# Cobalt-27/CompactFusion

Measured on AMD Instinct MI355X. Metric: residual_compressed_activation_exchange_throughput, higher is better.
Workload: dtype f16

## Files before the change

compactfusion_amd/csrc/cfx_absmean.hip:

```cpp
#include <hip/hip_runtime.h>
#include <hip/hip_ext.h>
#include <stdint.h>
#include <stdio.h>
#include <stdlib.h>
#include <string.h>
#include <algorithm>
#include "cfx.h"
#include "cfx_internal.h"
#include "cfx_device.h"
#include "cfx_host.h"

#define CFX_I_FLAG_LR_FACTORS_ONLY 0x100
#define CFX_I_FLAG_LR_ABS 0x200
extern "C" CFX_HIDDEN size_t cfx_i_lr_workspace_bytes_any(int N, int C, int rank, int batch);
extern "C" CFX_HIDDEN void cfx_i_lr_factor_offsets(int N, int C, int rank, size_t* offU16, size_t* offV16, size_t* per);

template <bool EMIT_BITS, int US, bool WT = false, int NW = WAVES, bool PUB = false, bool KEEP = false, bool TAG = false>
__device__ __forceinline__ void absmean_stats_body(const cfx_comp_item& it, int N, int C, int R, int CB, int bx, int by,
                                                   u64* rowpart, u64 (*sm)[TILE_C], Probe probe = Probe(),
                                                   h16x8* xk = nullptr, h16x8* bk = nullptr, TagArena ta = TagArena()) {
#define SSTAMP(k) probe.at(k)
    const TileCoord t = tile_coord_at(bx, by, N, C, R);
    const int cb = bx;
    u64* colpart = rowpart + (size_t)N * CB;
// ... 250 lines not shown
        for (int e = 0; e < 8; ++e) acc[j][e] = 0.f;
    for (int k0 = 0; k0 < K; k0 += 8) {
        h16 v[8][8];
#pragma unroll
        for (int e = 0; e < 8; ++e)
#pragma unroll
            for (int k = 0; k < 8; ++k) v[e][k] = (k0 + k < K) ? VT[(size_t)(t.c + e) * K + k0 + k] : (h16)0;
#pragma unroll
        for (int j = 0; j < RPT; ++j) {
            const int r = t.r0 + t.w + j * WAVES;
            if (r >= t.r1) continue;
            h16 u[8];
#pragma unroll
            for (int k = 0; k < 8; ++k) u[k] = (k0 + k < K) ? U[(size_t)r * K + k0 + k] : (h16)0;
#pragma unroll
            for (int e = 0; e < 8; ++e)
#pragma unroll
                for (int k = 0; k < 8; ++k) acc[j][e] += (float)(h16)(u[k] * v[e][k]);
        }
    }
#pragma unroll
    for (int j = 0; j < RPT; ++j) {
        const int r = t.r0 + t.w + j * WAVES;
        if (r >= t.r1) continue;
        h16x8 bv = (h16x8)(h16)0, xv = (h16x8)(h16)0;
        if (base) bv = ld8(base + (size_t)r * C + t.c);
        unsigned byte;
        if (QUANT) {
            xv = ld8(x + (size_t)r * C + t.c);
            const h16x8 d = xv - bv;
            byte = 0;
#pragma unroll
            for (int i = 0; i < 8; ++i) byte |= (d[i] >= (h16)0 ? 1u : 0u) << i;
            pk[(size_t)r * C8 + (t.c >> 3)] = (unsigned char)byte;
        } else byte = pk[(size_t)r * C8 + (t.c >> 3)];
        if (!upd) continue;
        h16x8 o;
#pragma unroll
        for (int e = 0; e < 8; ++e) {
            const h16 sc = (h16)acc[j][e];
            const h16 recv = ((byte >> e) & 1u) ? sc : -sc;
            o[e] = base ? (h16)(bv[e] + recv) : recv;
        }
        if (QUANT && !ef) o = xv;
        st8(out + (size_t)r * C + t.c, o);
    }
}

#ifndef WATCH_SLEEP
#define WATCH_SLEEP 4
#endif
#ifndef INT2_FLAG_SLEEP
#define INT2_FLAG_SLEEP 2
#endif
__device__ __forceinline__ void scales_watch(const TagArena& ta, int N, int C, int c0, int r0, long long timeout) {
    const int tid = threadIdx.x;
    if (tid < 2) {
        const u64* w = tid ? ta.tU + min(r0, N - 1) : ta.tV + min(c0 + ((r0 >> 1) & (TILE_C - 1)), C - 1);
        SpinClock clk;
        while (!tag_is(ld_wt(w), ta.tagbits)) {
            __builtin_amdgcn_s_sleep(WATCH_SLEEP);
            if (clk.expired(timeout)) break;
        }
    }
    lds_barrier();
}
template <int ROWS, bool WATCH = true>
__device__ __forceinline__ bool scales_from_tagged(const TagArena& ta, int N, int C, int c0, int r0, u16* s16, long long timeout, unsigned* err) {
    static_assert(ROWS <= TILE_C, "one token word per thread (512 threads = the column block's channels)");
    const int tid = threadIdx.x;
    const u64* pv = ta.tV + min(c0 + tid, C - 1);
    const u64* pu = ta.tU + min(r0 + tid, N - 1);
    SpinClock clk;
    if (WATCH) scales_watch(ta, N, C, c0, r0, timeout);
    for (;;) {
        const u64 v = ld_wt(pv);
        const u64 u = tid < ROWS ? ld_wt(pu) : ta.tagbits;
        const bool ok = tag_is(v, ta.tagbits) && tag_is(u, ta.tagbits);
        s16[tid] = (u16)v;
        if (tid < ROWS) s16[TILE_C + tid] = (u16)u;
        if (!__syncthreads_or(ok ? 0 : 1)) return true;
        __builtin_amdgcn_s_sleep(2);
        if (__syncthreads_or(!ok && clk.expired(timeout) ? 1 : 0)) {
            if (tid == 0) gate_fail(err);
            return false;
        }
    }
}

#ifndef ONEBIT_D_TAGGED
#define ONEBIT_D_TAGGED 0
#endif
template <int NW, int KR, int KL, bool ST>
__device__ __forceinline__ void binary_dequant_gated_body(const cfx_decomp_item& it, int N, int C, int R, int tile_x, int tile_y,
                                                         unsigned* gate, unsigned expect, unsigned* err, long long timeout, u32x4* lds,
                                                         Probe probe = Probe(), bool remote = false, bool tagged = false, TagArena ta = TagArena(),
                                                         u16* s16 = nullptr) {
    constexpr int K = KR + KL;
#define GSTAMP(k) do { if (ST && probe.on()) { asm volatile("s_waitcnt vmcnt(0)" ::: "memory"); probe.at(k); } } while (0)
    const TileCoord t = tile_coord_at(tile_x, tile_y, N, C, R);
    if (ST) { probe.at(0); probe.set(7, 4); }
    const unsigned char* pk = (const unsigned char*)it.packet;
    const int C8 = C >> 3;
    const u16* U = (const u16*)(pk + (size_t)N * C8);
    const u16* V = U + N;
    const h16* base = (const h16*)it.base;
    h16* out = (h16*)it.recon;
    const int cc = min(t.c, C - 8);
    h16x8 bv[KR];
    if (base) {
#pragma unroll
        for (int j = 0; j < KR; ++j) bv[j] = ld8nt(base + (size_t)min(t.r0 + t.w + NW * j, t.r1 - 1) * C + cc);
        if constexpr (KL > 0) {
            h16x8 tl[KL > 0 ? KL : 1];
#pragma unroll
            for (int j = 0; j < KL; ++j) tl[j] = ld8nt(base + (size_t)min(t.r0 + t.w + NW * (KR + j), t.r1 - 1) * C + cc);
#pragma unroll
            for (int j = 0; j < KL; ++j) lds[j * (NW * 64) + threadIdx.x] = __builtin_bit_cast(u32x4, tl[j]);
        }
    } else {
#pragma unroll
        for (int j = 0; j < KR; ++j) bv[j] = (h16x8)(h16)0;
    }
    GSTAMP(1);
    h16x8 v8;
    u16 ul;
    unsigned by[K];
    if (tagged) {
        scales_watch(ta, N, C, tile_x * TILE_C, t.r0, timeout);
        if (ST) probe.at(2);
#pragma unroll
        for (int j = 0; j < K; ++j) by[j] = ld_wt(pk + (size_t)min(t.r0 + t.w + NW * j, t.r1 - 1) * C8 + (cc >> 3));
        if (!scales_from_tagged<NW * K, false>(ta, N, C, tile_x * TILE_C, t.r0, s16, timeout, err)) return;
        v8 = __builtin_bit_cast(h16x8, *(const u16x8*)(s16 + 8 * t.lane));
        ul = s16[TILE_C + min(t.w + NW * min(t.lane, K - 1), t.r1 - 1 - t.r0)];
    } else if (!gate_wait<true>(gate, expect, err, timeout)) return;
    else if (remote) {
        if (ST) probe.at(2);
        u16x8 vb;
#pragma unroll
        for (int i = 0; i < 8; ++i) vb[i] = ld_sys(V + cc + i);
        v8 = __builtin_bit_cast(h16x8, vb);
        ul = ld_sys(U + min(t.r0 + t.w + NW * min(t.lane, K - 1), t.r1 - 1));
#pragma unroll
        for (int j = 0; j < K; ++j) by[j] = ld_sys(pk + (size_t)min(t.r0 + t.w + NW * j, t.r1 - 1) * C8 + (cc >> 3));
    } else {
        if (ST) probe.at(2);
        v8 = ld8_wt(V + cc);
        ul = ld_wt(U + min(t.r0 + t.w + NW * min(t.lane, K - 1), t.r1 - 1));
#pragma unroll
        for (int j = 0; j < K; ++j) by[j] = ld_wt(pk + (size_t)min(t.r0 + t.w + NW * j, t.r1 - 1) * C8 + (cc >> 3));
    }
    GSTAMP(3);
#pragma unroll
    for (int j = 0; j < K; ++j) {
        const int rr = t.r0 + t.w + NW * j;
        const h16 uj = hfrom((u16)__builtin_amdgcn_readlane((int)ul, j));
        if (rr < t.r1 && t.act) {
            const h16x8 s = v8 * uj;
            u16x8 sb = __builtin_bit_cast(u16x8, s);
#pragma unroll
            for (int i = 0; i < 8; ++i) sb[i] ^= ((by[j] >> i) & 1u) ? (u16)0 : (u16)0x8000;
            const h16x8 recv = __builtin_bit_cast(h16x8, sb);
            h16x8 bj = (h16x8)(h16)0;
            if (j < KR) bj = bv[j < KR ? j : 0];
            else if (base) bj = __builtin_bit_cast(h16x8, lds[(j - KR) * (NW * 64) + threadIdx.x]);
            st8nt(out + (size_t)rr * C + t.c, base ? (bj + recv) : recv);
        }
    }
    GSTAMP(4);
#undef GSTAMP
}

__device__ __forceinline__ void row_sums2_wt(const u64* rowpart, const unsigned* row32, int N, int CB, int m0, int m1, bool two, u64& s0, u64& s1) {
    s0 = 0; s1 = 0;
    for (int k0 = 0; k0 < CB; k0 += FUSED_RCH) {
        unsigned a[FUSED_RCH], b[FUSED_RCH];
#pragma unroll
        for (int j = 0; j < FUSED_RCH; ++j) a[j] = ld_wt(&row32[(size_t)min(k0 + j, CB - 1) * N + m0]);
        if (two) {
#pragma unroll
            for (int j = 0; j < FUSED_RCH; ++j) b[j] = ld_wt(&row32[(size_t)min(k0 + j, CB - 1) * N + m1]);
        } else {
#pragma unroll
            for (int j = 0; j < FUSED_RCH; ++j) b[j] = 0;
        }
        bool sat = false;
#pragma unroll
        for (int j = 0; j < FUSED_RCH; ++j) {
            s0 += (k0 + j < CB) ? a[j] : 0; s1 += (k0 + j < CB) ? b[j] : 0;
            sat |= (a[j] == PART_SAT) | (b[j] == PART_SAT);
        }
        if (sat) {
            for (int j = 0; j < FUSED_RCH && k0 + j < CB; ++j) {
                if (a[j] == PART_SAT) s0 += ld_wt(&rowpart[(size_t)(k0 + j) * N + m0]) - (u64)PART_SAT;
                if (two && b[j] == PART_SAT) s1 += ld_wt(&rowpart[(size_t)(k0 + j) * N + m1]) - (u64)PART_SAT;
            }
        }
    }
}

template <bool GATED>
__device__ __forceinline__ void absmean_last_arriver_jobs(const cfx_comp_item& it, int N, int C, int CB, int P, int bx, u64* rowpart,
                                                          unsigned* tick, int per_byte, int eps_mode, u64 (*sm)[TILE_C], bool last_col,
                                                          bool last_all, Probe probe, unsigned* gate, unsigned gate_expect) {
    constexpr int NT = FUSED_NT;
#define STAMP(k) probe.at(k)
    lds_barrier();
    const int tid = threadIdx.x;
    const u64* colpart = rowpart + (size_t)N * CB;
    const unsigned* row32 = part32_of(rowpart, N, C, CB);
    const unsigned* col32 = row32 + (size_t)N * CB;
    h16* U = (h16*)((char*)it.packet + (size_t)N * (C / per_byte));
    h16* V = U + N;
    const int c = bx * TILE_C + tid;
    const int cc = min(c, C - 1);
    unsigned v[FUSED_CH];
    if (last_col) {
#pragma unroll
        for (int j = 0; j < FUSED_CH; ++j) v[j] = ld_wt(&col32[(size_t)min(j, P - 1) * C + cc]);
    }
    u64 keep0 = 0, keep1 = 0;
    if (last_all) row_sums2_wt(rowpart, row32, N, CB, min(tid, N - 1), min(tid + NT, N - 1), (tid & ~63) + NT < N, keep0, keep1);
    asm volatile("" ::: "memory");
    STAMP(4);
    u64* smem = &sm[1][0];
    float m0 = 0.f, m1 = 0.f;
    if (last_all) {
        const h16 h0 = mean16(keep0, C), h1 = mean16(keep1, C);
        m0 = (float)h0; m1 = (float)h1;
        u64 acc = 0;
        if (tid < N) acc += habs_units(hbits(h0));
        if (tid + NT < N) acc += habs_units(hbits(h1));
        for (int n0 = tid + 2 * NT; n0 - tid < N; n0 += 2 * NT) {
            const int n1 = n0 + NT;
            u64 s0, s1;
            row_sums2_wt(rowpart, row32, N, CB, min(n0, N - 1), min(n1, N - 1), (n1 & ~63) < N, s0, s1);
            if (n0 < N) acc += habs_units(hbits(mean16(s0, C)));
            if (n1 < N) acc += habs_units(hbits(mean16(s1, C)));
        }
        STAMP(13);
        u64 wtot;
        if (N <= 2 * NT) {
            const unsigned lo = wave_sum_u32_dpp((unsigned)(acc & 0xffffffu));
            const unsigned hi = wave_sum_u32_dpp((unsigned)(acc >> 24));
            wtot = ((u64)hi << 24) + lo;
        } else wtot = wave_sum_u64(acc);
        STAMP(14);
        if ((tid & 63) == 0) smem[tid >> 6] = wtot;
    }
    h16 vmean = (h16)0;
    if (last_col) {
        u64 a = 0;
        for (int p0 = 0; p0 < P; p0 += FUSED_CH) {
            if (p0) {
#pragma unroll
                for (int j = 0; j < FUSED_CH; ++j) v[j] = ld_wt(&col32[(size_t)min(p0 + j, P - 1) * C + cc]);
            }
            bool sat = false;
#pragma unroll
            for (int j = 0; j < FUSED_CH; ++j) { a += (p0 + j < P) ? v[j] : 0; sat |= v[j] == PART_SAT; }
            if (sat) {
                for (int j = 0; j < FUSED_CH && p0 + j < P; ++j)
                    if (v[j] == PART_SAT) a += ld_wt(&colpart[(size_t)(p0 + j) * C + cc]) - (u64)PART_SAT;
            }
        }
        vmean = mean16(a, N);
    }
    STAMP(5);
    if (last_all) {
        lds_barrier();
        STAMP(15);
        u64 tot = 0;
#pragma unroll
        for (int w = 0; w < NT / 64; ++w) tot += smem[w];
        const h16 mu = mean16(tot, N);
        const float den = eps_mode ? (float)(h16)((float)mu + 1e-6f) : (float)mu;
#define PUT16(ptr, val) do { const h16 _v = (val); if (GATED) st_wt((u16*)(ptr), hbits(_v)); else *(ptr) = _v; } while (0)
        if (tid < N) PUT16(&U[tid], (h16)(m0 / den));
        if (tid + NT < N) PUT16(&U[tid + NT], (h16)(m1 / den));
        for (int n0 = tid + 2 * NT; n0 - tid < N; n0 += 2 * NT) {
            const int n1 = n0 + NT;
            u64 s0, s1;
            row_sums2_wt(rowpart, row32, N, CB, min(n0, N - 1), min(n1, N - 1), (n1 & ~63) < N, s0, s1);
            if (n0 < N) PUT16(&U[n0], (h16)((float)mean16(s0, C) / den));
            if (n1 < N) PUT16(&U[n1], (h16)((float)mean16(s1, C) / den));
        }
        if (tid == 0) st_wt(tick + TICK_ALL, 0u);
    }
    if (last_col) {
        if (c < C) PUT16(&V[c], vmean);
        if (tid == 0) st_wt(tick + 1 + bx, 0u);
    }
#undef PUT16
    if (GATED) {
        asm volatile("s_waitcnt vmcnt(0)" ::: "memory");
        lds_barrier();
        if (tid == 0) gate_arrive_few(gate, (last_all ? 1u : 0u) + (last_col ? 1u : 0u));
    }
    STAMP(6);
#undef STAMP
}

__device__ __forceinline__ void absmean_tagged_jobs(const cfx_comp_item& it, int N, int C, int CB, int P, int bx, u64* rowpart, const TagArena& ta,
                                                    int per_byte, int eps_mode, u64 (*sm)[TILE_C], bool do_col, bool do_row, Probe probe,
                                                    unsigned* gate, unsigned* err, long long timeout) {
    constexpr int NT = FUSED_NT;
#define STAMP(k) probe.at(k)
    lds_barrier();
    const int tid = threadIdx.x;
    const u64* colpart = rowpart + (size_t)N * CB;
    h16* U = (h16*)((char*)it.packet + (size_t)N * (C / per_byte));
    h16* V = U + N;
    SpinClock clk;
    bool failed = false;
#define PUT16(ptr, val) st_wt((u16*)(ptr), hbits(val))
    if (do_col) {
        const int c = bx * TILE_C + tid, cc = min(c, C - 1);
        u64 a = 0;
        for (int p0 = 0; p0 < P && !failed; p0 += FUSED_CH) {
            u64 v[FUSED_CH];
            for (;;) {
#pragma unroll
                for (int j = 0; j < FUSED_CH; ++j) v[j] = ld_wt(&ta.tcol[(size_t)min(p0 + j, P - 1) * C + cc]);
                bool ok = true;
#pragma unroll
                for (int j = 0; j < FUSED_CH; ++j) ok = ok && tag_is(v[j], ta.tagbits);
                if (ok) break;
                __builtin_amdgcn_s_sleep(2);
                if (clk.expired(timeout)) { failed = true; break; }
            }
#pragma unroll
            for (int j = 0; j < FUSED_CH; ++j) {
                const u64 w = v[j] & TAG_SAT;
                if (p0 + j < P) a += (w == TAG_SAT && !failed) ? ld_wt(&colpart[(size_t)(p0 + j) * C + cc]) : w;
            }
        }
        STAMP(4);
        failed = __syncthreads_or(failed ? 1 : 0) != 0;
        if (!failed) {
            if (c < C) {
                const h16 vm = mean16(a, N);
                st_wt(&ta.tV[c], ta.tagbits | (u64)hbits(vm));
                PUT16(&V[c], vm);
            }
            asm volatile("s_waitcnt vmcnt(0)" ::: "memory");
            lds_barrier();
            if (tid == 0) gate_arrive_few(gate, 1u);
        }
        STAMP(5);
    }
    if (do_row && !failed) {
        u64* smem = &sm[1][0];
        auto row_sum = [&](int n) {
            const int nc = min(n, N - 1);
            u64 s_ = 0;
            for (int k0 = 0; k0 < CB && !failed; k0 += FUSED_RCH) {
                u64 q[FUSED_RCH];
                for (;;) {
#pragma unroll
                    for (int j = 0; j < FUSED_RCH; ++j) q[j] = ld_wt(&ta.trow[(size_t)min(k0 + j, CB - 1) * N + nc]);
                    bool ok = true;
#pragma unroll
                    for (int j = 0; j < FUSED_RCH; ++j) ok = ok && tag_is(q[j], ta.tagbits);
                    if (ok) break;
                    __builtin_amdgcn_s_sleep(2);
                    if (clk.expired(timeout)) { failed = true; break; }
                }
#pragma unroll
                for (int j = 0; j < FUSED_RCH; ++j) {
                    const u64 w = q[j] & TAG_SAT;
                    if (k0 + j < CB) s_ += (w == TAG_SAT && !failed) ? ld_wt(&rowpart[(size_t)(k0 + j) * N + nc]) : w;
                }
            }
            return s_;
        };
        h16 h0 = (h16)0, h1 = (h16)0;
        u64 acc = 0;
        for (int n0 = tid, i = 0; n0 - tid < N; n0 += NT, ++i) {
            const h16 h = mean16(row_sum(n0), C);
            if (i == 0) h0 = h;
            if (i == 1) h1 = h;
            if (n0 < N) acc += habs_units(hbits(h));
        }
        STAMP(13);
        const u64 wtot = wave_sum_u64(acc);
        if ((tid & 63) == 0) smem[tid >> 6] = wtot;
        failed = __syncthreads_or(failed ? 1 : 0) != 0;
        STAMP(15);
        if (!failed) {
            u64 tot = 0;
#pragma unroll
            for (int w = 0; w < NT / 64; ++w) tot += smem[w];
            const h16 mu = mean16(tot, N);
            const float den = eps_mode ? (float)(h16)((float)mu + 1e-6f) : (float)mu;
            for (int n0 = tid, i = 0; n0 < N; n0 += NT, ++i) {
                const h16 h = i == 0 ? h0 : (i == 1 ? h1 : mean16(row_sum(n0), C));
                const h16 un = (h16)((float)h / den);
                st_wt(&ta.tU[n0], ta.tagbits | (u64)hbits(un));
                PUT16(&U[n0], un);
            }
            asm volatile("s_waitcnt vmcnt(0)" ::: "memory");
            lds_barrier();
            if (tid == 0) gate_arrive_few(gate, 1u);
        }
        STAMP(6);
    }
#undef PUT16
#undef STAMP
    if (failed && tid == 0) gate_fail(err);
}

template <int US>
__device__ __forceinline__ void own_tile_finish(const cfx_comp_item& it, int N, int C, int R, int bx, int by, int flags, const h16x8* xk,
                                                const h16x8* bk, unsigned* gate1, unsigned expect1, unsigned* gate2, unsigned expect2,
                                                unsigned* err, long long timeout, unsigned char* smw, const TagArena& ta, u16* s16) {
    constexpr int NW = FUSED_NW;
    static_assert(US * 8 <= 64, "a wave publishes its US rows of codes with 8 lanes a row");
    const TileCoord t = tile_coord_at(bx, by, N, C, R);
    h16* nb = (h16*)it.new_base;
    const bool upd = (flags & CFX_FLAG_UPDATE_CACHE) && nb;
    const bool ef = !(flags & CFX_FLAG_NO_EF);
    unsigned char* pk = (unsigned char*)it.packet;
    (void)gate1; (void)expect1;
    if (!scales_from_tagged<NW * US>(ta, N, C, bx * TILE_C, t.r0, s16, timeout, err)) return;
    const h16x8 ch8 = __builtin_bit_cast(h16x8, *(const u16x8*)(s16 + 8 * t.lane));
    const u16 ul = s16[TILE_C + min(t.w + NW * min(t.lane, US - 1), t.r1 - 1 - t.r0)];
    const bool has_base = it.base != nullptr;
    u16 codes[US];
#pragma unroll
    for (int j = 0; j < US; ++j) {
        const int rr = t.r0 + t.w + NW * j;
        const h16 tk = hfrom((u16)__builtin_amdgcn_readlane((int)ul, j));
        codes[j] = 0;
        if (rr < t.r1 && t.act) {
            const h16x8 d = xk[j] - bk[j];
            const h16x8 thr = ch8 * tk;
            const h16x8 a = habs8(d);
            unsigned code = 0;
#pragma unroll
            for (int i = 0; i < 8; ++i) {
                const unsigned sg = d[i] >= (h16)0 ? 1u : 0u;
                const unsigned m = a[i] > thr[i] ? 1u : 0u;
                code |= ((sg << 1) | m) << (2 * i);
            }
            codes[j] = (u16)code;
            ((u16*)smw)[j * 64 + t.lane] = (u16)code;
        }
    }
    {
        const int j = t.lane >> 3, seg = t.lane & 7;
        const int rr = t.r0 + t.w + NW * j;
        if (t.lane < 8 * US && rr < t.r1 && bx * TILE_C + seg * 64 < C)
            st16_wt(pk + (size_t)rr * (C >> 2) + bx * (TILE_C >> 2) + seg * 16, *(const u32x4*)(smw + j * 128 + seg * 16));
    }
    asm volatile("s_waitcnt vmcnt(0)" ::: "memory");
    lds_barrier();
    if (threadIdx.x == 0) {
        st_wt(&ta.tdone[(size_t)bx * ((N + R - 1) / R) + by], ta.tagbits);
        gate_arrive(gate2, 1u, expect2);
    }
    if (upd) {
#pragma unroll
        for (int j = 0; j < US; ++j) {
            const int rr = t.r0 + t.w + NW * j;
            const h16 tk = hfrom((u16)__builtin_amdgcn_readlane((int)ul, j));
            if (rr < t.r1 && t.act) {
                const h16x8 recv = int2_recv(codes[j], ch8 * tk);
                st8nt(nb + (size_t)rr * C + t.c, ef ? (has_base ? (bk[j] + recv) : recv) : xk[j]);
            }
        }
    }
}

template <bool EMIT_BITS, int US, bool GATED = false, bool KEEP = false>
__device__ __forceinline__ void absmean_fused_body(const cfx_comp_item& it, int N, int C, int R, int CB, int P, int bx, int by,
                                                   u64* rowpart, unsigned* tick, int per_byte, int eps_mode, u64 (*sm)[TILE_C], int dbg,
                                                   Probe probe, unsigned* gate = nullptr, unsigned gate_expect = 0, int flags = 0,
                                                   unsigned* gate2 = nullptr, unsigned expect2 = 0, unsigned* err = nullptr, long long timeout = 0,
                                                   TagArena ta = TagArena()) {
#define STAMP(k) probe.at(k)
    STAMP(0);
#ifdef CFX_DEV_PROBES
    if (dbg == 3) return;
    if (dbg == 4) {
        const TileCoord t = tile_coord_at(bx, by, N, C, R);
        h16x8 acc = (h16x8)(h16)0;
        for (int r = t.r0 + t.w; r < t.r1; r += FUSED_NW * US) {
            h16x8 xv[US], bv[US];
#pragma unroll
            for (int j = 0; j < US; ++j) {
                const int rr = min(r + FUSED_NW * j, t.r1 - 1);
                xv[j] = ld8nt((const h16*)it.x + (size_t)rr * C + min(t.c, C - 8));
                bv[j] = ld8((const h16*)it.base + (size_t)rr * C + min(t.c, C - 8));
            }
#pragma unroll
            for (int j = 0; j < US; ++j) acc += xv[j] - bv[j];
        }
        if (acc[0] == (h16)12345.0f) ((h16*)it.packet)[threadIdx.x] = acc[1];
        return;
    }
#endif
    h16x8 xk[KEEP ? US : 1], bk[KEEP ? US : 1];
    absmean_stats_body<EMIT_BITS, US, true, FUSED_NW, GATED, KEEP, GATED>(it, N, C, R, CB, bx, by, rowpart, sm, probe, xk, bk, ta);
    STAMP(1);
    if constexpr (GATED) {
        const bool v_wg = by == P - 1;
        const bool u_wg = P >= 2 ? (by == P - 2 && bx == CB - 1) : (bx == CB - 1);
        probe.copy(2, 1); probe.copy(3, 1); probe.set(7, (v_wg ? 1 : 0) | (u_wg ? 2 : 0));
        if (v_wg || u_wg) {
            u32x4* park = (u32x4*)&sm[FUSED_NW][0];
            if constexpr (KEEP) {
                park[threadIdx.x] = __builtin_bit_cast(u32x4, xk[US - 1]);
                park[FUSED_NT + threadIdx.x] = __builtin_bit_cast(u32x4, bk[US - 1]);
            }
            absmean_tagged_jobs(it, N, C, CB, P, bx, rowpart, ta, per_byte, eps_mode, sm, v_wg, u_wg, probe, gate, err, timeout);
            if constexpr (KEEP) {
                xk[US - 1] = __builtin_bit_cast(h16x8, park[threadIdx.x]);
                bk[US - 1] = __builtin_bit_cast(h16x8, park[FUSED_NT + threadIdx.x]);
            }
        }
    } else {
    asm volatile("s_waitcnt vmcnt(0)" ::: "memory");
    __syncthreads();
    STAMP(2);
#ifdef CFX_DEV_PROBES
    if (dbg == 1) return;
#endif
    unsigned* flag = (unsigned*)&sm[0][0];
    if (threadIdx.x == 0) flag[0] = __hip_atomic_fetch_add(tick + 1 + bx, 1u, __ATOMIC_RELAXED, __HIP_MEMORY_SCOPE_AGENT);
    if (threadIdx.x == 64) (void)__hip_atomic_fetch_add(tick + TICK_ALL, 1u, __ATOMIC_RELAXED, __HIP_MEMORY_SCOPE_AGENT);
    lds_barrier();
    const bool last_col = flag[0] == (unsigned)(P - 1);
    const bool u_wg = bx == 0 && by == 0;
    STAMP(3);
    probe.set(7, (last_col ? 1 : 0) | (u_wg ? 2 : 0));
#ifdef CFX_DEV_PROBES
    if (dbg == 2) {
        if (last_col && threadIdx.x == 0) st_wt(tick + 1 + bx, 0u);
        if (u_wg && threadIdx.x == 0) {
            while (ld_wt(tick + TICK_ALL) != (unsigned)(CB * P)) __builtin_amdgcn_s_sleep(1);
            st_wt(tick + TICK_ALL, 0u);
        }
        return;
    }
#endif
    if (last_col)
        absmean_last_arriver_jobs<GATED>(it, N, C, CB, P, bx, rowpart, tick, per_byte, eps_mode, sm, true, false, probe, gate, gate_expect);
    if (u_wg) {
        bool failed = false;
        if (threadIdx.x == 0) {
            SpinClock clk;
            while (ld_wt(tick + TICK_ALL) != (unsigned)(CB * P)) {
                __builtin_amdgcn_s_sleep(1);
                if (clk.expired(timeout)) { failed = true; gate_fail(err); break; }
            }
        }
        if (__syncthreads_or(failed ? 1 : 0)) return;
        absmean_last_arriver_jobs<GATED>(it, N, C, CB, P, bx, rowpart, tick, per_byte, eps_mode, sm, false, true, probe, gate, gate_expect);
    }
    }
    if constexpr (KEEP)
        own_tile_finish<US>(it, N, C, R, bx, by, flags, xk, bk, gate, gate_expect, gate2, expect2, err, timeout,
                                       (unsigned char*)&sm[__builtin_amdgcn_readfirstlane(threadIdx.x >> 6)][0], ta, (u16*)&sm[FUSED_NW + 4][0]);
#undef STAMP
}

struct FusedArgs {
    int N, C, CB, R, P;
    int n_st;
    int dq_R, dq_rb;
    int per_byte, eps_mode;
    int dbg;
    u64* ws;
    size_t ws_stride;
    unsigned* tick;
    Probe probe;
    int n_g, g_R, g_rb, n_gt;
    unsigned* gate;
    unsigned gate_expect;
    unsigned* gate_err;
    long long timeout;
    u64* tarena; size_t tarena_stride; unsigned tag;
    signed char src[CFX_MAX_BATCH];
    unsigned* xgate;
    unsigned xexpect;
    int remote;
    P2PInline p2p;
};
#ifndef GATE_WPE
#define GATE_WPE 4
#endif
template <bool EMIT_BITS, int US, bool GATED = false, bool ST = false>
__global__ __launch_bounds__(FUSED_NT, GATE_WPE) __attribute__((amdgpu_num_vgpr(52))) void k_absmean_compress(BatchC batch, BatchD ride, BatchD gated, FusedArgs a) {
    __shared__ u64 sm[FUSED_NW][TILE_C];
    int b = blockIdx.x;
    if (b < a.n_st) {
        const int per = a.CB * a.P;
        const int z = b / per, rem = b - z * per;
        const int by = rem / a.CB;
        absmean_fused_body<EMIT_BITS, US, GATED>(batch.it[z], a.N, a.C, a.R, a.CB, a.P, rem - by * a.CB, by, a.ws + (size_t)z * a.ws_stride,
                                                 a.tick + z * TICK_WORDS, a.per_byte, a.eps_mode, sm, a.dbg,
                                                 a.probe.of(b), a.gate, a.gate_expect, 0, nullptr, 0u, a.gate_err, a.timeout,
                                                 tag_arena_of(a.tarena, a.tarena_stride, z, a.N, a.C, a.CB, a.P, a.tag));
        if constexpr (GATED) {
            if (b == 0 && a.p2p.own) p2p_exchange_inline(a.gate, a.gate_expect, 1, a.p2p, a.xgate, a.xexpect, a.gate_err);
        }
        return;
    }
    if constexpr (EMIT_BITS) {
        b -= a.n_st;
        if constexpr (GATED) {
            if (b < a.n_g) {
                const int per = a.CB * a.g_rb;
                for (int t = b; t < a.n_gt; t += a.n_g) {
                    const int item = t / per, rem = t - item * per;
                    const int ty = rem / a.CB;
                    const int sz = a.src[item];
                    const TagArena ta = tag_arena_of(a.tarena, a.tarena_stride, sz >= 0 ? sz : 0, a.N, a.C, a.CB, a.P, a.tag);
                    binary_dequant_gated_body<FUSED_NW, GATE_KR, 0, ST>(gated.it[item], a.N, a.C, a.g_R, rem - ty * a.CB, ty, a.xgate ? a.xgate : a.gate,
                                                                a.xgate ? a.xexpect : a.gate_expect, a.gate_err, a.timeout,
                                                                nullptr,
                                                                a.probe.of(blockIdx.x), a.remote != 0 && sz < 0,
                                                                ONEBIT_D_TAGGED && sz >= 0, ta, (u16*)&sm[0][0]);
                }
                return;
            }
            b -= a.n_g;
        }
        const int per = a.CB * a.dq_rb;
        const int item = b / per, rem = b - item * per;
        const int ty = rem / a.CB;
        binary_dequant_body<FUSED_NW>(ride.it[item], a.N, a.C, a.dq_R, rem - ty * a.CB, ty);
    }
}

#ifndef PIPE_US
#define PIPE_US 2
#endif
#define PIPE_MAX_DQ CFX_PIPE_MAX_DQ
struct BatchDX { cfx_decomp_item it[PIPE_MAX_DQ]; };
struct PipeArgs {
    int N, C, CB;
    int n_fin, fin_bpi, fin_P;
    int n_st, st_R, st_P;
    int dq_R, dq_rb;
    const u64* ws_fin;
    u64* ws_st;
    size_t ws_stride;
};
template <bool STEADY>
__global__ __launch_bounds__(NTHR) __attribute__((amdgpu_waves_per_eu(8, 8))) void k_binary_pipe(BatchDX dq, BatchC fin, BatchC st, PipeArgs a) {
    __shared__ u64 sm[WAVES][TILE_C];
    int b = blockIdx.x;
    if (b < a.n_fin) {
        const int item = b / a.fin_bpi;
        absmean_finalize_body<NTHR>(fin.it[item], a.N, a.C, a.CB, a.fin_P, 8, 0, a.ws_fin + (size_t)item * a.ws_stride, b - item * a.fin_bpi, &sm[0][0]);
        return;
    }
    b -= a.n_fin;
    if (b < a.n_st) {
        const int per = a.CB * a.st_P;
        const int item = b / per, rem = b - item * per;
        const int ty = rem / a.CB;
        absmean_stats_body<true, PIPE_US>(st.it[item], a.N, a.C, a.st_R, a.CB, rem - ty * a.CB, ty, a.ws_st + (size_t)item * a.ws_stride, sm);
        return;
    }
    b -= a.n_st;
    const int per = a.CB * a.dq_rb;
    const int item = b / per, rem = b - item * per;
    const int ty = rem / a.CB;
    binary_dequant_body<WAVES>(dq.it[item], a.N, a.C, a.dq_R, rem - ty * a.CB, ty);
}


__global__ __launch_bounds__(NTHR) void k_int2_quant(BatchC batch, int N, int C, int R, int flags) {
    const cfx_comp_item it = batch.it[blockIdx.z];
    const TileCoord t = tile_coord(N, C, R);
    const int C4 = C >> 2;
    unsigned char* pk = (unsigned char*)it.packet;
    const h16* TOK = (const h16*)(pk + (size_t)N * C4);
    const h16* CH = TOK + N;
    const h16* x = (const h16*)it.x;
    const h16* base = (const h16*)it.base;
    h16* nb = (h16*)it.new_base;
    const bool upd = (flags & CFX_FLAG_UPDATE_CACHE) && nb;
    const bool ef = !(flags & CFX_FLAG_NO_EF);
    const bool al16 = (((uintptr_t)CH) & 15) == 0;
    h16x8 ch8 = (h16x8)(h16)0;
    if (t.act) ch8 = ld8_tail(CH + t.c, al16);

    for (int r = t.r0 + t.w; r < t.r1; r += WAVES * UNROLL) {
        h16x8 xv[UNROLL], bv[UNROLL];
        h16 tk[UNROLL];
#pragma unroll
        for (int j = 0; j < UNROLL; ++j) {
            const int rr = r + WAVES * j;
            xv[j] = (h16x8)(h16)0; bv[j] = (h16x8)(h16)0; tk[j] = (h16)0;
            if (rr < t.r1 && t.act) {
                xv[j] = ld8nt(x + (size_t)rr * C + t.c);
                if (base) bv[j] = ld8nt(base + (size_t)rr * C + t.c);
                tk[j] = TOK[rr];
            }
        }
#pragma unroll
        for (int j = 0; j < UNROLL; ++j) {
            const int rr = r + WAVES * j;
            if (rr < t.r1 && t.act) {
                const h16x8 d = xv[j] - bv[j];
                const h16x8 thr = ch8 * tk[j];
                const h16x8 a = habs8(d);
                unsigned code = 0;
#pragma unroll
                for (int i = 0; i < 8; ++i) {
                    const unsigned s = d[i] >= (h16)0 ? 1u : 0u;
                    const unsigned m = a[i] > thr[i] ? 1u : 0u;
                    code |= ((s << 1) | m) << (2 * i);
                }
                *reinterpret_cast<u16*>(pk + (size_t)rr * C4 + (t.c >> 2)) = (u16)code;
                if (upd) {
                    h16x8 o;
                    if (ef) {
                        const h16x8 recv = int2_recv((u16)code, thr);
                        o = base ? (bv[j] + recv) : recv;
                    } else {
                        o = xv[j];
                    }
                    st8nt(nb + (size_t)rr * C + t.c, o);
                }
            }
        }
    }
}

__global__ __launch_bounds__(NTHR) void k_int2_dequant(BatchD batch, int N, int C, int R, unsigned* pre, unsigned pre_val) {
    if (pre && (blockIdx.x | blockIdx.y | blockIdx.z | threadIdx.x) == 0) st_wt(pre, pre_val);
    const cfx_decomp_item it = batch.it[blockIdx.z];
    const TileCoord t = tile_coord(N, C, R);
    const int C4 = C >> 2;
    const unsigned char* pk = (const unsigned char*)it.packet;
    const h16* TOK = (const h16*)(pk + (size_t)N * C4);
    const h16* CH = TOK + N;
    const h16* base = (const h16*)it.base;
    h16* out = (h16*)it.recon;
    const bool al16 = (((uintptr_t)CH) & 15) == 0;
    h16x8 ch8 = (h16x8)(h16)0;
    if (t.act) ch8 = ld8_tail(CH + t.c, al16);

    for (int r = t.r0 + t.w; r < t.r1; r += WAVES * UNROLL) {
        h16x8 bv[UNROLL];
        u16 cd[UNROLL];
        h16 tk[UNROLL];
#pragma unroll
        for (int j = 0; j < UNROLL; ++j) {
            const int rr = r + WAVES * j;
            bv[j] = (h16x8)(h16)0; cd[j] = 0; tk[j] = (h16)0;
            if (rr < t.r1 && t.act) {
                if (base) bv[j] = ld8nt(base + (size_t)rr * C + t.c);
                cd[j] = *reinterpret_cast<const u16*>(pk + (size_t)rr * C4 + (t.c >> 2));
                tk[j] = TOK[rr];
            }
        }
#pragma unroll
        for (int j = 0; j < UNROLL; ++j) {
            const int rr = r + WAVES * j;
            if (rr < t.r1 && t.act) {
                const h16x8 thr = ch8 * tk[j];
                const h16x8 recv = int2_recv(cd[j], thr);
                st8nt(out + (size_t)rr * C + t.c, base ? (bv[j] + recv) : recv);
            }
        }
    }
}

template <int NW, int KR, int KL>
__device__ __forceinline__ void int2_dequant_gated_body(const cfx_decomp_item& it, int N, int C, int R, int tile_x, int tile_y,
                                                       unsigned* gate, unsigned expect, unsigned* err, long long timeout, u32x4* lds,
                                                       unsigned* xgate = nullptr, unsigned xexpect = 0, bool remote = false,
                                                       bool tagged = false, TagArena ta = TagArena(), int Rs = 0, u16* s16 = nullptr) {
    constexpr int K = KR + KL;
    const TileCoord t = tile_coord_at(tile_x, tile_y, N, C, R);
    const int C4 = C >> 2;
    const unsigned char* pk = (const unsigned char*)it.packet;
    const u16* TOK = (const u16*)(pk + (size_t)N * C4);
    const u16* CH = TOK + N;
    const h16* base = (const h16*)it.base;
    h16* out = (h16*)it.recon;
    const int cc = min(t.c, C - 8);
    h16x8 bv[KR];
    if (base) {
#pragma unroll
        for (int j = 0; j < KR; ++j) bv[j] = ld8nt(base + (size_t)min(t.r0 + t.w + NW * j, t.r1 - 1) * C + cc);
        if constexpr (KL > 0) {
            h16x8 tl[KL > 0 ? KL : 1];
#pragma unroll
            for (int j = 0; j < KL; ++j) tl[j] = ld8nt(base + (size_t)min(t.r0 + t.w + NW * (KR + j), t.r1 - 1) * C + cc);
#pragma unroll
            for (int j = 0; j < KL; ++j) lds[j * (NW * 64) + threadIdx.x] = __builtin_bit_cast(u32x4, tl[j]);
        }
    } else {
#pragma unroll
        for (int j = 0; j < KR; ++j) bv[j] = (h16x8)(h16)0;
    }
    h16x8 ch8;
    u16 ul;
    u16 cd[K];
    if (tagged) {
        bool failed = false;
        if (t.w == 0) {
            const int P = (N + Rs - 1) / Rs, by0 = t.r0 / Rs, by1 = (t.r1 - 1) / Rs;
            const u64* f = ta.tdone + (size_t)tile_x * P;
            SpinClock clk;
            for (;;) {
                const u64 v = by0 + t.lane <= by1 ? ld_wt(f + by0 + t.lane) : ta.tagbits;
                if (__builtin_amdgcn_ballot_w64(!tag_is(v, ta.tagbits)) == 0) break;
                __builtin_amdgcn_s_sleep(INT2_FLAG_SLEEP);
                if (clk.expired(timeout)) { failed = true; if (t.lane == 0) gate_fail(err); break; }
            }
        }
// ... 462 lines not shown
```

Baseline: 2138.

## Stage U/V scales in LDS for 16-byte stores, pair row sums, gate tagged scales

The U and V scale outputs are now staged in LDS and written with aligned 16-byte write-through stores instead of one 2-byte store per thread. The row-sum pass now handles two rows per thread per iteration, so the tag polls and partial loads for both rows are issued together. Tagged copies of the scales (tU/tV) are written only when a template flag (KEEP or ONEBIT_D_TAGGED) asks for them. The cost is extra LDS barriers and staging, the staged loop overwrites LDS that other code may rely on, and if a tagged-scale consumer is missing from the flag condition it could hang.

Result: no change. 2145 (median of 6 runs) (+0.3%).

```diff
diff --git a/compactfusion_amd/csrc/cfx_absmean.hip b/compactfusion_amd/csrc/cfx_absmean.hip
--- a/compactfusion_amd/csrc/cfx_absmean.hip
+++ b/compactfusion_amd/csrc/cfx_absmean.hip
@@ -576,19 +576,34 @@
 #undef STAMP
 }
 
+__device__ __forceinline__ void st_scales16_wt(u16* dst, const u16* s16, int n) {
+    const int tid = threadIdx.x;
+    const int head = min(n, (int)(((16u - ((unsigned)(uintptr_t)dst & 15u)) & 15u) >> 1));
+    const int body = (n - head) & ~7, tail = n - head - body;
+    for (int g = tid; g < body >> 3; g += FUSED_NT) {
+        u16x8 w;
+#pragma unroll
+        for (int i = 0; i < 8; ++i) w[i] = s16[head + 8 * g + i];
+        st16_wt(dst + head + 8 * g, __builtin_bit_cast(u32x4, w));
+    }
+    if (tid < head) st_wt(dst + tid, s16[tid]);
+    if (tid >= 8 && tid - 8 < tail) st_wt(dst + head + body + (tid - 8), s16[head + body + (tid - 8)]);
+}
+template <bool TSCALES>
 __device__ __forceinline__ void absmean_tagged_jobs(const cfx_comp_item& it, int N, int C, int CB, int P, int bx, u64* rowpart, const TagArena& ta,
                                                     int per_byte, int eps_mode, u64 (*sm)[TILE_C], bool do_col, bool do_row, Probe probe,
                                                     unsigned* gate, unsigned* err, long long timeout) {
     constexpr int NT = FUSED_NT;
+    constexpr int STAGE = TILE_C * 4;
 #define STAMP(k) probe.at(k)
     lds_barrier();
     const int tid = threadIdx.x;
     const u64* colpart = rowpart + (size_t)N * CB;
-    h16* U = (h16*)((char*)it.packet + (size_t)N * (C / per_byte));
-    h16* V = U + N;
+    u16* U = (u16*)((char*)it.packet + (size_t)N * (C / per_byte));
+    u16* V = U + N;
+    u16* s16 = (u16*)&sm[0][0];
     SpinClock clk;
     bool failed = false;
-#define PUT16(ptr, val) st_wt((u16*)(ptr), hbits(val))
     if (do_col) {
         const int c = bx * TILE_C + tid, cc = min(c, C - 1);
         u64 a = 0;
@@ -613,11 +628,12 @@
         STAMP(4);
         failed = __syncthreads_or(failed ? 1 : 0) != 0;
         if (!failed) {
-            if (c < C) {
-                const h16 vm = mean16(a, N);
-                st_wt(&ta.tV[c], ta.tagbits | (u64)hbits(vm));
-                PUT16(&V[c], vm);
-            }
+            const int nc = min(TILE_C, C - bx * TILE_C);
+            const h16 vm = mean16(a, N);
+            if (TSCALES && c < C) st_wt(&ta.tV[c], ta.tagbits | (u64)hbits(vm));
+            if (tid < nc) s16[tid] = hbits(vm);
+            lds_barrier();
+            st_scales16_wt(V + bx * TILE_C, s16, nc);
             asm volatile("s_waitcnt vmcnt(0)" ::: "memory");
             lds_barrier();
             if (tid == 0) gate_arrive_few(gate, 1u);
@@ -626,36 +642,48 @@
     }
     if (do_row && !failed) {
         u64* smem = &sm[1][0];
-        auto row_sum = [&](int n) {
-            const int nc = min(n, N - 1);
-            u64 s_ = 0;
+        auto row_sum2 = [&](int m0, int m1, bool two, u64& s0, u64& s1) {
+            const int a0 = min(m0, N - 1), a1 = min(m1, N - 1);
+            s0 = 0; s1 = 0;
             for (int k0 = 0; k0 < CB && !failed; k0 += FUSED_RCH) {
-                u64 q[FUSED_RCH];
+                u64 q[FUSED_RCH], r[FUSED_RCH];
                 for (;;) {
 #pragma unroll
-                    for (int j = 0; j < FUSED_RCH; ++j) q[j] = ld_wt(&ta.trow[(size_t)min(k0 + j, CB - 1) * N + nc]);
+                    for (int j = 0; j < FUSED_RCH; ++j) q[j] = ld_wt(&ta.trow[(size_t)min(k0 + j, CB - 1) * N + a0]);
+                    if (two) {
+#pragma unroll
+                        for (int j = 0; j < FUSED_RCH; ++j) r[j] = ld_wt(&ta.trow[(size_t)min(k0 + j, CB - 1) * N + a1]);
+                    } else {
+#pragma unroll
+                        for (int j = 0; j < FUSED_RCH; ++j) r[j] = ta.tagbits;
+                    }
                     bool ok = true;
 #pragma unroll
-                    for (int j = 0; j < FUSED_RCH; ++j) ok = ok && tag_is(q[j], ta.tagbits);
+                    for (int j = 0; j < FUSED_RCH; ++j) ok = ok && tag_is(q[j], ta.tagbits) && tag_is(r[j], ta.tagbits);
                     if (ok) break;
                     __builtin_amdgcn_s_sleep(2);
                     if (clk.expired(timeout)) { failed = true; break; }
                 }
 #pragma unroll
                 for (int j = 0; j < FUSED_RCH; ++j) {
-                    const u64 w = q[j] & TAG_SAT;
-                    if (k0 + j < CB) s_ += (w == TAG_SAT && !failed) ? ld_wt(&rowpart[(size_t)(k0 + j) * N + nc]) : w;
+                    const u64 w = q[j] & TAG_SAT, x = r[j] & TAG_SAT;
+                    if (k0 + j < CB) {
+                        s0 += (w == TAG_SAT && !failed) ? ld_wt(&rowpart[(size_t)(k0 + j) * N + a0]) : w;
+                        s1 += (x == TAG_SAT && !failed && two) ? ld_wt(&rowpart[(size_t)(k0 + j) * N + a1]) : x;
+                    }
                 }
             }
-            return s_;
         };
         h16 h0 = (h16)0, h1 = (h16)0;
         u64 acc = 0;
-        for (int n0 = tid, i = 0; n0 - tid < N; n0 += NT, ++i) {
-            const h16 h = mean16(row_sum(n0), C);
-            if (i == 0) h0 = h;
-            if (i == 1) h1 = h;
-            if (n0 < N) acc += habs_units(hbits(h));
+        for (int n0 = tid; n0 - tid < N; n0 += 2 * NT) {
+            const bool two = n0 - tid + (tid & ~63) + NT < N;
+            u64 s0, s1;
+            row_sum2(n0, n0 + NT, two, s0, s1);
+            const h16 a = mean16(s0, C), b = mean16(s1, C);
+            if (n0 == tid) { h0 = a; h1 = b; }
+            if (n0 < N) acc += habs_units(hbits(a));
+            if (n0 + NT < N) acc += habs_units(hbits(b));
         }
         STAMP(13);
         const u64 wtot = wave_sum_u64(acc);
@@ -668,11 +696,21 @@
             for (int w = 0; w < NT / 64; ++w) tot += smem[w];
             const h16 mu = mean16(tot, N);
             const float den = eps_mode ? (float)(h16)((float)mu + 1e-6f) : (float)mu;
-            for (int n0 = tid, i = 0; n0 < N; n0 += NT, ++i) {
-                const h16 h = i == 0 ? h0 : (i == 1 ? h1 : mean16(row_sum(n0), C));
-                const h16 un = (h16)((float)h / den);
-                st_wt(&ta.tU[n0], ta.tagbits | (u64)hbits(un));
-                PUT16(&U[n0], un);
+            for (int b0 = 0; b0 < N; b0 += STAGE) {
+                if (b0) lds_barrier();
+                for (int n0 = b0 + tid; n0 < min(N, b0 + STAGE); n0 += NT) {
+                    h16 h = n0 == tid ? h0 : h1;
+                    if (n0 >= tid + 2 * NT) {
+                        u64 s0, s1;
+                        row_sum2(n0, n0, false, s0, s1);
+                        h = mean16(s0, C);
+                    }
+                    const h16 un = (h16)((float)h / den);
+                    if (TSCALES) st_wt(&ta.tU[n0], ta.tagbits | (u64)hbits(un));
+                    s16[n0 - b0] = hbits(un);
+                }
+                lds_barrier();
+                st_scales16_wt(U + b0, s16, min(STAGE, N - b0));
             }
             asm volatile("s_waitcnt vmcnt(0)" ::: "memory");
             lds_barrier();
@@ -680,7 +718,6 @@
         }
         STAMP(6);
     }
-#undef PUT16
 #undef STAMP
     if (failed && tid == 0) gate_fail(err);
 }
@@ -788,7 +825,7 @@
                 park[threadIdx.x] = __builtin_bit_cast(u32x4, xk[US - 1]);
                 park[FUSED_NT + threadIdx.x] = __builtin_bit_cast(u32x4, bk[US - 1]);
             }
-            absmean_tagged_jobs(it, N, C, CB, P, bx, rowpart, ta, per_byte, eps_mode, sm, v_wg, u_wg, probe, gate, err, timeout);
+            absmean_tagged_jobs<KEEP || ONEBIT_D_TAGGED>(it, N, C, CB, P, bx, rowpart, ta, per_byte, eps_mode, sm, v_wg, u_wg, probe, gate, err, timeout);
             if constexpr (KEEP) {
                 xk[US - 1] = __builtin_bit_cast(h16x8, park[threadIdx.x]);
                 bk[US - 1] = __builtin_bit_cast(h16x8, park[FUSED_NT + threadIdx.x]);
```
